# hpcaitech/Open-Sora

Hardware: NVIDIA H100
Metric: denoise-steps/sec STDiT3-XL/2 64x32x32 bf16 (higher is better)
Workload: dtype bf16

## Files before the change

### open-sora_b200/csrc/gemm_sm90.cu

```cuda
#include <stdlib.h>

#include <type_traits>

#include "common.cuh"
#include "tiles.cuh"
#include "wgmma.cuh"

namespace osb {

constexpr int kBlockM = 128;
constexpr int kBlockK = 64;
constexpr int kNumThreads = 384;
constexpr int kStageBudget = 200 * 1024;
constexpr int kSmemLimit = 227 * 1024;

enum { kPlain = 0, kConv = 1, kHeadTiles = 2, kLora = 3, kText = 4, kFp8 = 5, kFp8Blk = 6 };

struct Fp8BlockParams {
  int64_t a_ld, a_kstride;
  uint8_t* d8;
  float* d_scale;
  int64_t ldd8, ld_dscale;
};

// ... 23 lines not shown
  const float* sin;
};

struct ConvGeom {
  int32_t wt_log2, ht_log2;
  int32_t tiles_w, tiles_h, tiles_t, nb;
  int32_t w_out, h_out, t_out;
  int32_t sw, sh, st;
  int32_t kw_n, kh_n;
  int32_t cin_chunks;
};

__host__ __device__ constexpr bool staged_epilogue(int mode) { return mode == kPlain || mode == kConv || mode == kLora || mode == kFp8 || mode == kFp8Blk; }

template <int BLOCK_N, bool kStaged = false>
struct GemmCfg {
  static constexpr int A_BYTES = kBlockM * kBlockK * 2;
  static constexpr int B_BYTES = BLOCK_N * kBlockK * 2;
  static constexpr int STAGE_BYTES = A_BYTES + B_BYTES;
  static constexpr int EPI_BYTES = kStaged ? kBlockM * BLOCK_N * 2 : 0;
  static constexpr int RING_BUDGET = kStaged ? kSmemLimit - 1024 - 256 - EPI_BYTES : kStageBudget;
  static constexpr int STAGES_RAW = RING_BUDGET / STAGE_BYTES;
  static constexpr int STAGES = STAGES_RAW > 6 ? 6 : STAGES_RAW;
  static constexpr int NUM_BARS = 2 * STAGES + (kStaged ? 1 : 0);
  static constexpr int SMEM_BYTES = STAGES * STAGE_BYTES + EPI_BYTES + 1024 + 8 * NUM_BARS;
  static_assert(STAGES >= 2, "pipeline needs at least two stages");
  static_assert(SMEM_BYTES <= kSmemLimit, "shared memory");
  static_assert(B_BYTES % 1024 == 0, "W tile must keep 1024-byte swizzle-atom alignment");
  static_assert(BLOCK_N % 16 == 0 && BLOCK_N <= 256, "wgmma N");
  static_assert(!kStaged || BLOCK_N % 64 == 0, "the staged epilogue moves 64-column boxes");
};

template <int BLOCK_N, int kMode>
__global__ void __launch_bounds__(kNumThreads, 1)
gemm_bf16_kernel(const __grid_constant__ CUtensorMap tmap_a, const __grid_constant__ CUtensorMap tmap_w,
                 const GemmEpilogueParams p, const ConvGeom cg, const HeadTileParams ht,
                 const __grid_constant__ CUtensorMap tmap_u, const __grid_constant__ CUtensorMap tmap_lb,
                 const int32_t lora_k_blocks,
                 const float* a_scale, const float* w_scale,
                 const Fp8BlockParams fb,
                 const __grid_constant__ CUtensorMap tmap_r,
                 const __grid_constant__ CUtensorMap tmap_d) {
  constexpr bool kStaged = staged_epilogue(kMode);
  using Cfg = GemmCfg<BLOCK_N, kStaged>;
  constexpr int kStages = Cfg::STAGES;
  constexpr int kBK = (kMode == kFp8 || kMode == kFp8Blk) ? 2 * kBlockK : kBlockK;
  constexpr uint32_t kEpiBoxBytes = kBlockM * 128;

  extern __shared__ uint8_t smem_raw[];
  const uint32_t smem_base = (smem_u32(smem_raw) + 1023u) & ~1023u;
  const uint32_t epi_base = smem_base + kStages * Cfg::STAGE_BYTES;
  const uint32_t bar_base = epi_base + Cfg::EPI_BYTES;
  auto full_bar = [&](int s) { return bar_base + 8u * s; };
  auto empty_bar = [&](int s) { return bar_base + 8u * (kStages + s); };
  const uint32_t res_bar = bar_base + 8u * (2 * kStages);
  auto smem_a = [&](int s) { return smem_base + s * Cfg::STAGE_BYTES; };
  auto smem_b = [&](int s) { return smem_base + s * Cfg::STAGE_BYTES + Cfg::A_BYTES; };

  const int wg = threadIdx.x >> 7;
  const int tid_wg = threadIdx.x & 127;
  const int64_t num_n_blocks = (p.N + BLOCK_N - 1) / BLOCK_N;
  const int64_t m_blk = blockIdx.x / num_n_blocks, n_blk = blockIdx.x % num_n_blocks;
  const int64_t num_k_blocks = (p.K + kBK - 1) / kBK;
  const int64_t total_k_blocks = kMode == kLora ? num_k_blocks + lora_k_blocks : num_k_blocks;
  int n_i = 0, t0 = 0, h0 = 0, w0 = 0;
  if constexpr (kMode == kConv) {
    const int tw = (int)(m_blk % cg.tiles_w);
    const int th = (int)((m_blk / cg.tiles_w) % cg.tiles_h);
    const int tt = (int)((m_blk / ((int64_t)cg.tiles_w * cg.tiles_h)) % cg.tiles_t);
    n_i = (int)(m_blk / ((int64_t)cg.tiles_w * cg.tiles_h * cg.tiles_t));
    w0 = tw << cg.wt_log2;
    h0 = th << cg.ht_log2;
    t0 = tt * (128 >> (cg.wt_log2 + cg.ht_log2));
  }

  if (threadIdx.x == 0) {
    tma_prefetch_desc(&tmap_a);
    tma_prefetch_desc(&tmap_w);
    if constexpr (kMode == kLora) {
      tma_prefetch_desc(&tmap_u);
      tma_prefetch_desc(&tmap_lb);
    }
    if constexpr (kStaged) {
      if (p.R != nullptr) tma_prefetch_desc(&tmap_r);
      tma_prefetch_desc(&tmap_d);
      mbar_init(res_bar, 1);
    }
    for (int s = 0; s < kStages; ++s) {
      mbar_init(full_bar(s), 1);
      mbar_init(empty_bar(s), 2);
    }
    fence_barrier_init();
  }
  __syncthreads();
  pdl_wait();

  if (wg == 0) {
    if (tid_wg == 0) {
      const int32_t a_row = (int32_t)(m_blk * kBlockM);
      const int32_t w_row = (int32_t)(n_blk * BLOCK_N);
      if constexpr (kStaged) {
        if (p.R != nullptr) {
          const int live = (int)min((int64_t)(BLOCK_N / 64), (p.N - w_row + 63) / 64);
          mbar_expect_tx(res_bar, (uint32_t)live * kEpiBoxBytes);
          for (int c = 0; c < live; ++c) {
            if constexpr (kMode == kConv)
              tma_load_5d(&tmap_r, res_bar, epi_base + c * kEpiBoxBytes, w_row + 64 * c, w0, h0, t0, n_i);
            else
              tma_load_2d(&tmap_r, res_bar, epi_base + c * kEpiBoxBytes, w_row + 64 * c, a_row);
          }
        }
      }
      int stage = 0;
      uint32_t phase = 0;
      for (int64_t kb = 0; kb < num_k_blocks; ++kb) {
        mbar_wait_notrace(empty_bar(stage), phase ^ 1);
        const int32_t k0 = (int32_t)(kb * kBK);
        mbar_expect_tx(full_bar(stage), Cfg::STAGE_BYTES);
        if constexpr (kMode == kConv) {
          const int tap = (int)(kb / cg.cin_chunks);
          const int32_t ac = (int32_t)(kb - (int64_t)tap * cg.cin_chunks) * kBlockK;
          const int32_t aw = w0 * cg.sw + tap % cg.kw_n;
          const int32_t ah = h0 * cg.sh + (tap / cg.kw_n) % cg.kh_n;
          const int32_t at = t0 * cg.st + tap / (cg.kw_n * cg.kh_n);
          tma_load_5d(&tmap_a, full_bar(stage), smem_a(stage), ac, aw, ah, at, n_i);
        } else {
          tma_load_2d(&tmap_a, full_bar(stage), smem_a(stage), k0, a_row);
        }
        tma_load_2d(&tmap_w, full_bar(stage), smem_b(stage), k0, w_row);
        if (++stage == kStages) { stage = 0; phase ^= 1; }
      }
      if constexpr (kMode == kLora) {
        for (int32_t lk = 0; lk < lora_k_blocks; ++lk) {
          mbar_wait_notrace(empty_bar(stage), phase ^ 1);
          mbar_expect_tx(full_bar(stage), Cfg::STAGE_BYTES);
          tma_load_2d(&tmap_u, full_bar(stage), smem_a(stage), lk * kBlockK, a_row);
          tma_load_2d(&tmap_lb, full_bar(stage), smem_b(stage), lk * kBlockK, w_row);
          if (++stage == kStages) { stage = 0; phase ^= 1; }
        }
      }
      pdl_launch_dependents();
    }
    return;
  }

  const int cw = wg - 1;
  float acc[BLOCK_N / 2];
#pragma unroll
  for (int i = 0; i < BLOCK_N / 2; ++i) acc[i] = 0.f;
  if constexpr (kMode == kFp8 || kMode == kFp8Blk) {
    float part[BLOCK_N / 2];
#pragma unroll
    for (int i = 0; i < BLOCK_N / 2; ++i) part[i] = 0.f;
    const float* sa_row0 = a_scale;
    const float* sa_row1 = a_scale;
    if constexpr (kMode == kFp8Blk) {
      const int64_t r0 = m_blk * kBlockM + cw * 64 + (tid_wg >> 5) * 16 + ((tid_wg & 31) >> 2);
      sa_row0 = a_scale + min(r0, p.M - 1) * fb.a_ld;
      sa_row1 = a_scale + min(r0 + 8, p.M - 1) * fb.a_ld;
    }
    int stage = 0;
    uint32_t phase = 0;
    for (int64_t kb = 0; kb < total_k_blocks; ++kb) {
      float s0 = 1.f, s1 = 1.f;
      if constexpr (kMode == kFp8Blk) {
        s0 = __ldg(sa_row0 + kb * fb.a_kstride);
        s1 = __ldg(sa_row1 + kb * fb.a_kstride);
      }
      mbar_wait_notrace(full_bar(stage), phase);
      const uint64_t da = make_sw128_kmajor_desc(smem_a(stage) + (uint32_t)(cw * 64 * 128));
      const uint64_t db = make_sw128_kmajor_desc(smem_b(stage));
      wgmma_fence_regs(part);
      wgmma_fence();
#pragma unroll
      for (int k = 0; k < 4; ++k)
        WgmmaFp8<BLOCK_N>::mma(part, da + (uint64_t)(2 * k), db + (uint64_t)(2 * k), k > 0 ? 1u : 0u);
      wgmma_commit();
      wgmma_wait<0>();
      wgmma_fence_regs(part);
      if (tid_wg == 0) mbar_arrive(empty_bar(stage));
      if constexpr (kMode == kFp8Blk) {
#pragma unroll
        for (int j = 0; j < BLOCK_N / 8; ++j) {
          acc[4 * j] = fmaf(part[4 * j], s0, acc[4 * j]);
          acc[4 * j + 1] = fmaf(part[4 * j + 1], s0, acc[4 * j + 1]);
          acc[4 * j + 2] = fmaf(part[4 * j + 2], s1, acc[4 * j + 2]);
          acc[4 * j + 3] = fmaf(part[4 * j + 3], s1, acc[4 * j + 3]);
        }
      } else {
#pragma unroll
        for (int i = 0; i < BLOCK_N / 2; ++i) acc[i] += part[i];
      }
      if (++stage == kStages) { stage = 0; phase ^= 1; }
    }
  } else {
    int stage = 0, prev = 0;
    uint32_t phase = 0;
    for (int64_t kb = 0; kb < total_k_blocks; ++kb) {
      mbar_wait_notrace(full_bar(stage), phase);
      const uint64_t da = make_sw128_kmajor_desc(smem_a(stage) + (uint32_t)(cw * 64 * 128));
      const uint64_t db = make_sw128_kmajor_desc(smem_b(stage));
      wgmma_fence_regs(acc);
      wgmma_fence();
#pragma unroll
      for (int k = 0; k < kBlockK / 16; ++k)
        Wgmma<BLOCK_N>::mma(acc, da + (uint64_t)(2 * k), db + (uint64_t)(2 * k), (kb > 0 || k > 0) ? 1u : 0u);
      wgmma_commit();
      wgmma_wait<1>();
      wgmma_fence_regs(acc);
      if (kb > 0 && tid_wg == 0) mbar_arrive(empty_bar(prev));
      prev = stage;
      if (++stage == kStages) { stage = 0; phase ^= 1; }
    }
    wgmma_wait<0>();
    wgmma_fence_regs(acc);
  }

  const int warp_in = tid_wg >> 5, lane = tid_wg & 31;
  const int r_frag = cw * 64 + warp_in * 16 + (lane >> 2);
  const int c_frag = 2 * (lane & 3);

  if constexpr (kMode == kLora) {
    if (w_scale != nullptr) {
#pragma unroll
      for (int j = 0; j < BLOCK_N / 8; ++j) {
        const int64_t n = min(n_blk * BLOCK_N + 8 * j + c_frag, p.N - 2);
        const float2 cs = __ldg(reinterpret_cast<const float2*>(w_scale + n));
        acc[4 * j] *= cs.x;
        acc[4 * j + 1] *= cs.y;
        acc[4 * j + 2] *= cs.x;
        acc[4 * j + 3] *= cs.y;
      }
    }
  }

  if constexpr (kMode == kFp8Blk && BLOCK_N == 128) {
    if (p.epilogue == OSB_EPI_BIAS_GELU_TANH_FP8) {
      const int64_t n0 = n_blk * BLOCK_N + c_frag;
#pragma unroll
      for (int h = 0; h < 2; ++h) {
        const int64_t row = m_blk * kBlockM + r_frag + 8 * h;
        float amax = 0.f;
#pragma unroll
        for (int j = 0; j < BLOCK_N / 8; ++j) {
          const int64_t n = n0 + 8 * j;
          const float2 sw = __ldg(reinterpret_cast<const float2*>(w_scale + n));
          float v0 = acc[4 * j + 2 * h] * sw.x, v1 = acc[4 * j + 2 * h + 1] * sw.y;
          if (p.bias) {
            const float2 b = unpack_bf16x2(__ldg(reinterpret_cast<const uint32_t*>(p.bias + n)));
            v0 += b.x;
            v1 += b.y;
          }
          v0 = gelu_tanh(v0);
          v1 = gelu_tanh(v1);
          acc[4 * j + 2 * h] = v0;
          acc[4 * j + 2 * h + 1] = v1;
          amax = fmaxf(amax, fmaxf(fabsf(v0), fabsf(v1)));
        }
        amax = fmaxf(amax, __shfl_xor_sync(0xffffffffu, amax, 1));
        amax = fmaxf(amax, __shfl_xor_sync(0xffffffffu, amax, 2));
        const float s = amax > 0.f ? amax / 448.0f : 1.0f;
        if (row < p.M) {
          uint8_t* drow = fb.d8 + row * fb.ldd8;
#pragma unroll
          for (int j = 0; j < BLOCK_N / 8; ++j)
            *reinterpret_cast<uint16_t*>(drow + n0 + 8 * j) =
                (uint16_t)e4m3x2(acc[4 * j + 2 * h] / s, acc[4 * j + 2 * h + 1] / s);
          if (c_frag == 0) fb.d_scale[row * fb.ld_dscale + n_blk] = s;
        }
      }
      return;
    }
  }

  if constexpr (kMode == kHeadTiles) {
    constexpr int D = BLOCK_N / 2;
    using HT = HeadTileCfg<D>;
    constexpr int JH = D / 8;
    const int C = ht.heads * D;
    const uint32_t chunk_bytes = (uint32_t)ht.map.TR * 128u;
#pragma unroll
    for (int h = 0; h < 2; ++h) {
      const int64_t row = m_blk * kBlockM + r_frag + 8 * h;
      const bool row_ok = row < p.M;
      uint32_t pos = 0, tile_i = 0;
      int r = 0;
      if (row_ok) tile_of_row(ht.map, (uint32_t)row, tile_i, pos, r);
#pragma unroll
      for (int hh = 0; hh < 2; ++hh) {
        const int64_t col0 = n_blk * BLOCK_N + hh * D;
        if (col0 >= p.N) continue;
        const int kidx = (int)((uint32_t)col0 / (uint32_t)C);
        const int head = (int)((uint32_t)col0 - (uint32_t)kidx * (uint32_t)C) / D;
        const int kind = kidx % ht.nkinds;
        float x[JH][2];
#pragma unroll
        for (int j = 0; j < JH; ++j) {
          x[j][0] = acc[4 * (hh * JH + j) + 2 * h];
          x[j][1] = acc[4 * (hh * JH + j) + 2 * h + 1];
          if (p.bias) {
            const float2 b = unpack_bf16x2(__ldg(reinterpret_cast<const uint32_t*>(p.bias + col0 + 8 * j + c_frag)));
            x[j][0] += b.x;
            x[j][1] += b.y;
          }
        }
        if ((ht.norm_mask >> kind) & 1u) {
          float ss = 0.f;
#pragma unroll
          for (int j = 0; j < JH; ++j) ss += x[j][0] * x[j][0] + x[j][1] * x[j][1];
          ss += __shfl_xor_sync(0xffffffffu, ss, 1);
          ss += __shfl_xor_sync(0xffffffffu, ss, 2);
          const float rs = rsqrtf(ss * (1.0f / D) + ht.eps);
          const __nv_bfloat16* w = kind == 0 ? ht.norm_w[0] : (kind == 1 ? ht.norm_w[1] : (kind == 2 ? ht.norm_w[2] : ht.norm_w[3]));
#pragma unroll
          for (int j = 0; j < JH; ++j) {
            const float2 f = unpack_bf16x2(__ldg(reinterpret_cast<const uint32_t*>(w + 8 * j + c_frag)));
            x[j][0] *= rs * f.x;
            x[j][1] *= rs * f.y;
          }
        }
        if (!row_ok) continue;
        if ((ht.rope_mask >> kind) & 1u) {
#pragma unroll
          for (int j = 0; j < JH; ++j) {
            const int64_t i = (int64_t)pos * (D / 2) + (8 * j + c_frag) / 2;
            const float cc = __ldg(ht.cos + i), sn = __ldg(ht.sin + i);
            const float a = x[j][0], b = x[j][1];
            x[j][0] = a * cc - b * sn;
            x[j][1] = b * cc + a * sn;
          }
        }
        uint8_t* dst = ht.base + (int64_t)kidx * ht.kind_stride + (int64_t)head * ht.head_stride + (int64_t)tile_i * ht.tile_bytes;
#pragma unroll
        for (int j = 0; j < JH; ++j)
          *reinterpret_cast<uint32_t*>(dst + tile_unit_off<HT::MAIN>(r, j, chunk_bytes) + c_frag * 2) = pack_bf16x2(x[j][0], x[j][1]);
        if constexpr (HT::UP > HT::U)
          *reinterpret_cast<uint32_t*>(dst + tile_unit_off<HT::MAIN>(r, HT::U, chunk_bytes) + c_frag * 2) = 0u;
      }
    }
  } else if constexpr (kMode == kText) {
#pragma unroll
    for (int h = 0; h < 2; ++h) {
      const int64_t row = m_blk * kBlockM + r_frag + 8 * h;
      if (row >= p.M) continue;
      __nv_bfloat16* drow = p.D + row * p.ldd;
#pragma unroll
      for (int j = 0; j < BLOCK_N / 8; ++j) {
        const int64_t n = n_blk * BLOCK_N + 8 * j + c_frag;
        if (n >= p.N) continue;
        float v0 = acc[4 * j + 2 * h], v1 = acc[4 * j + 2 * h + 1];
        if (p.bias) {
          const float2 b = unpack_bf16x2(__ldg(reinterpret_cast<const uint32_t*>(p.bias + n)));
          v0 += b.x;
          v1 += b.y;
        }
        if (p.epilogue == OSB_EPI_GATED_GELU) {
          drow[n >> 1] = __float2bfloat16_rn(gelu_tanh(v0) * v1);
        } else {
          v0 = v0 / (1.0f + __expf(-1.702f * v0));
          v1 = v1 / (1.0f + __expf(-1.702f * v1));
          *reinterpret_cast<uint32_t*>(drow + n) = pack_bf16x2(v0, v1);
        }
      }
    }
  } else {
    static_assert(kStaged, "every other mode has its own epilogue");
    const float* gate_row[2] = {nullptr, nullptr};
    float sa[2] = {0.f, 0.f};
    if constexpr (kMode != kConv) {
      const uint32_t group_rows32 = (uint32_t)(p.group_rows > 0xffffffffll ? 0xffffffffu : p.group_rows);
#pragma unroll
      for (int h = 0; h < 2; ++h) {
        const int64_t row = min(m_blk * kBlockM + r_frag + 8 * h, p.M - 1);
        if (p.epilogue == OSB_EPI_BIAS_GATE_RES && p.gate != nullptr) {
          int64_t gi = (uint32_t)row / group_rows32;
          if (p.mod_index) gi = p.mod_index[gi];
          gate_row[h] = p.gate + gi * p.gate_stride;
        }
        if constexpr (kMode == kFp8) sa[h] = __ldg(a_scale + row);
      }
    }
    uint8_t* const epi = smem_raw + (epi_base - smem_u32(smem_raw));
    const bool gate_res = p.epilogue == OSB_EPI_BIAS_GATE_RES;
    if (!gate_res) gate_row[0] = gate_row[1] = nullptr;
    const bool has_res = gate_res && p.R != nullptr;
    if (p.R != nullptr) mbar_wait_notrace(res_bar, 0);
    auto body = [&](auto gelu) {
#pragma unroll
      for (int j = 0; j < BLOCK_N / 8; ++j) {
        const int64_t n = min(n_blk * BLOCK_N + 8 * j + c_frag, p.N - 2);
        float2 sw = make_float2(1.f, 1.f), b = make_float2(-0.f, -0.f);
        if constexpr (kMode == kFp8 || kMode == kFp8Blk) sw = __ldg(reinterpret_cast<const float2*>(w_scale + n));
        if (p.bias) b = unpack_bf16x2(__ldg(reinterpret_cast<const uint32_t*>(p.bias + n)));
#pragma unroll
        for (int h = 0; h < 2; ++h) {
          const int li = r_frag + 8 * h;
          uint32_t* const cell = reinterpret_cast<uint32_t*>(epi + (j >> 3) * kEpiBoxBytes + li * 128 +
                                                             (((j & 7) ^ (li & 7)) << 4) + c_frag * 2);
          float v0 = acc[4 * j + 2 * h], v1 = acc[4 * j + 2 * h + 1];
          if constexpr (kMode == kFp8) {
            v0 = __fmul_rn(v0, __fmul_rn(sa[h], sw.x));
            v1 = __fmul_rn(v1, __fmul_rn(sa[h], sw.y));
          } else if constexpr (kMode == kFp8Blk) {
            v0 = __fmul_rn(v0, sw.x);
            v1 = __fmul_rn(v1, sw.y);
          }
          v0 = __fadd_rn(v0, b.x);
          v1 = __fadd_rn(v1, b.y);
          if constexpr (decltype(gelu)::value) {
            v0 = gelu_tanh(v0);
            v1 = gelu_tanh(v1);
          } else {
            const float2 g = gate_row[h] ? __ldg(reinterpret_cast<const float2*>(gate_row[h] + n)) : make_float2(1.f, 1.f);
            const float2 rv = has_res ? unpack_bf16x2(*cell) : make_float2(-0.f, -0.f);
            v0 = __fadd_rn(__fmul_rn(v0, g.x), rv.x);
            v1 = __fadd_rn(__fmul_rn(v1, g.y), rv.y);
          }
          *cell = pack_bf16x2(v0, v1);
        }
      }
    };
    if (p.epilogue == OSB_EPI_BIAS_GELU_TANH)
      body(std::true_type{});
    else
      body(std::false_type{});
    fence_proxy_async_smem();
    named_barrier_sync(1, 256);
    if (threadIdx.x == 128) {
      const int32_t n0 = (int32_t)(n_blk * BLOCK_N);
      const int live = (int)min((int64_t)(BLOCK_N / 64), (p.N - n0 + 63) / 64);
      for (int c = 0; c < live; ++c) {
        if constexpr (kMode == kConv)
          tma_store_5d(&tmap_d, epi_base + c * kEpiBoxBytes, n0 + 64 * c, w0, h0, t0, n_i);
        else
          tma_store_2d(&tmap_d, epi_base + c * kEpiBoxBytes, n0 + 64 * c, (int32_t)(m_blk * kBlockM));
      }
      bulk_commit_group();
      bulk_wait_group_read_all();
    }
  }
}

template <int BLOCK_N, int kMode>
static int launch_kernel(const CUtensorMap& ta, const CUtensorMap& tw, const GemmEpilogueParams& p, const ConvGeom& cg,
                         const HeadTileParams& ht, int64_t tiles, cudaStream_t stream, const CUtensorMap* tu = nullptr,
                         const CUtensorMap* tlb = nullptr, int32_t lora_k_blocks = 0, const float* a_scale = nullptr,
                         const float* w_scale = nullptr, const Fp8BlockParams& fb = Fp8BlockParams{},
                         const CUtensorMap* tr = nullptr, const CUtensorMap* td = nullptr) {
  if (tiles >= (1ll << 31)) { set_error("osb gemm: too many output tiles (%lld)", (long long)tiles); return OSB_ERR_UNSUPPORTED; }
  cudaLaunchAttribute attr[2];
  cudaLaunchConfig_t cfg = launch_config(dim3((unsigned)tiles), dim3(kNumThreads),
                                         GemmCfg<BLOCK_N, staged_epilogue(kMode)>::SMEM_BYTES, stream, attr);
  OSB_CHECK_CUDA(cudaLaunchKernelEx(&cfg, gemm_bf16_kernel<BLOCK_N, kMode>, ta, tw, p, cg, ht, tu ? *tu : ta,
                                    tlb ? *tlb : tw, lora_k_blocks, a_scale, w_scale, fb, tr ? *tr : ta, td ? *td : ta));
  count_launch();
  return OSB_OK;
}

static int make_epilogue_maps(const GemmEpilogueParams& p, CUtensorMap* tr, CUtensorMap* td) {
  if (int rc = make_tmap_2d_bf16(td, p.D, p.M, p.N, p.ldd, kBlockM, 64)) return rc;
  if (p.R != nullptr) return make_tmap_2d_bf16(tr, p.R, p.M, p.N, p.ldr, kBlockM, 64);
  *tr = *td;
  return OSB_OK;
}

template <int D>
static int launch_gemm_ht(const osb_gemm_args& a, const HeadTileParams& ht, cudaStream_t stream) {
  constexpr int BLOCK_N = 2 * D;
  CUtensorMap ta, tw;
  int rc = make_tmap_2d_bf16(&ta, a.A, a.M, a.K, a.lda, kBlockM, kBlockK);
  if (rc) return rc;
  rc = make_tmap_2d_bf16(&tw, a.W, a.N, a.K, a.ldw, BLOCK_N, kBlockK);
  if (rc) return rc;
  GemmEpilogueParams p = {};
// ... 65 lines not shown
  if ((rc = init_one<128, kLora>())) return rc;
  if ((rc = init_one<192, kLora>())) return rc;
  if ((rc = init_one<256, kLora>())) return rc;
  if ((rc = init_one<64, kText>())) return rc;
  if ((rc = init_one<128, kText>())) return rc;
  if ((rc = init_one<192, kText>())) return rc;
  if ((rc = init_one<256, kText>())) return rc;
  if ((rc = init_one<64, kFp8>())) return rc;
  if ((rc = init_one<128, kFp8>())) return rc;
  if ((rc = init_one<64, kFp8Blk>())) return rc;
  if ((rc = init_one<128, kFp8Blk>())) return rc;
  return OSB_OK;
}

static int pick_block_n(int64_t M, int64_t N) {
  if (N <= 64) return 64;
  const int cands[3] = {256, 192, 128};
  int best = 256;
  int64_t best_cost = INT64_MAX;
  for (int i = 0; i < 3; ++i) {
    const int bn = cands[i];
    const int64_t tiles = ((M + kBlockM - 1) / kBlockM) * ((N + bn - 1) / bn);
    const int64_t waves = (tiles + sm_count() - 1) / sm_count();
    const int64_t cost = waves * bn;
    if (cost < best_cost) { best_cost = cost; best = bn; }
  }
  return best;
}

template <int BLOCK_N, int kMode = kFp8>
static int launch_gemm_fp8(const osb_gemm_fp8_args& a, cudaStream_t stream, const Fp8BlockParams& fb = Fp8BlockParams{}) {
  CUtensorMap ta, tw;
  int rc = make_tmap_2d_e4m3(&ta, a.A, a.M, a.K, a.lda, kBlockM, 2 * kBlockK);
  if (rc) return rc;
  rc = make_tmap_2d_e4m3(&tw, a.W, a.N, a.K, a.ldw, BLOCK_N, 2 * kBlockK);
  if (rc) return rc;
  GemmEpilogueParams p = {};
  p.bias = static_cast<const __nv_bfloat16*>(a.bias);
  p.D = static_cast<__nv_bfloat16*>(a.D);
  p.R = a.epilogue == OSB_EPI_BIAS_GATE_RES ? static_cast<const __nv_bfloat16*>(a.R) : nullptr;
  p.gate = a.gate;
  p.mod_index = a.mod_index;
  p.M = a.M; p.N = a.N; p.K = a.K;
  p.ldd = a.ldd;
  p.ldr = a.ldr;
  p.group_rows = a.group_rows > 0 ? a.group_rows : a.M;
  p.gate_stride = a.gate_stride;
// ... 302 lines not shown
```

Baseline: 11.20.

## Make SM90 GEMM persistent with overlapped epilogue and producer register rebalancing

Turns the one-tile-per-CTA GEMM into a persistent kernel: the grid is capped at the SM count and each CTA loops over tiles. The producer warp loads the next tile's K-blocks while the consumers run the previous epilogue, using a new epi_free barrier to guard the staged-epilogue buffer. The producer warpgroup gives up registers via setmaxnreg and the consumers take more. The head-tile epilogue now packs values with lane shuffles into 16-byte stores. The block-N cost model adds a per-tile overhead term. This hides launch and epilogue latency at the price of more synchronisation complexity and possible tile-scheduling imbalance.

Measured after the change: 11.94 (median of 6 runs). 6.6% higher.

```diff
diff --git a/open-sora_b200/csrc/gemm_sm90.cu b/open-sora_b200/csrc/gemm_sm90.cu
--- a/open-sora_b200/csrc/gemm_sm90.cu
+++ b/open-sora_b200/csrc/gemm_sm90.cu
@@ -69,7 +69,7 @@
   static constexpr int RING_BUDGET = kStaged ? kSmemLimit - 1024 - 256 - EPI_BYTES : kStageBudget;
   static constexpr int STAGES_RAW = RING_BUDGET / STAGE_BYTES;
   static constexpr int STAGES = STAGES_RAW > 6 ? 6 : STAGES_RAW;
-  static constexpr int NUM_BARS = 2 * STAGES + (kStaged ? 1 : 0);
+  static constexpr int NUM_BARS = 2 * STAGES + (kStaged ? 2 : 0);
   static constexpr int SMEM_BYTES = STAGES * STAGE_BYTES + EPI_BYTES + 1024 + 8 * NUM_BARS;
   static_assert(STAGES >= 2, "pipeline needs at least two stages");
   static_assert(SMEM_BYTES <= kSmemLimit, "shared memory");
@@ -101,25 +101,35 @@
   auto full_bar = [&](int s) { return bar_base + 8u * s; };
   auto empty_bar = [&](int s) { return bar_base + 8u * (kStages + s); };
   const uint32_t res_bar = bar_base + 8u * (2 * kStages);
+  const uint32_t epi_free = bar_base + 8u * (2 * kStages + 1);
   auto smem_a = [&](int s) { return smem_base + s * Cfg::STAGE_BYTES; };
   auto smem_b = [&](int s) { return smem_base + s * Cfg::STAGE_BYTES + Cfg::A_BYTES; };
 
   const int wg = threadIdx.x >> 7;
   const int tid_wg = threadIdx.x & 127;
   const int64_t num_n_blocks = (p.N + BLOCK_N - 1) / BLOCK_N;
-  const int64_t m_blk = blockIdx.x / num_n_blocks, n_blk = blockIdx.x % num_n_blocks;
+  const int64_t num_m_blocks =
+      kMode == kConv ? (int64_t)cg.nb * cg.tiles_t * cg.tiles_h * cg.tiles_w : (p.M + kBlockM - 1) / kBlockM;
+  const int64_t num_tiles = num_m_blocks * num_n_blocks;
   const int64_t num_k_blocks = (p.K + kBK - 1) / kBK;
   const int64_t total_k_blocks = kMode == kLora ? num_k_blocks + lora_k_blocks : num_k_blocks;
-  int n_i = 0, t0 = 0, h0 = 0, w0 = 0;
-  if constexpr (kMode == kConv) {
-    const int tw = (int)(m_blk % cg.tiles_w);
-    const int th = (int)((m_blk / cg.tiles_w) % cg.tiles_h);
-    const int tt = (int)((m_blk / ((int64_t)cg.tiles_w * cg.tiles_h)) % cg.tiles_t);
-    n_i = (int)(m_blk / ((int64_t)cg.tiles_w * cg.tiles_h * cg.tiles_t));
-    w0 = tw << cg.wt_log2;
-    h0 = th << cg.ht_log2;
-    t0 = tt * (128 >> (cg.wt_log2 + cg.ht_log2));
-  }
+  struct Tile {
+    int64_t m_blk, n_blk;
+    int n_i, t0, h0, w0;
+  };
+  auto tile_at = [&](int64_t t) {
+    Tile tl = {t / num_n_blocks, t % num_n_blocks, 0, 0, 0, 0};
+    if constexpr (kMode == kConv) {
+      const int tw = (int)(tl.m_blk % cg.tiles_w);
+      const int th = (int)((tl.m_blk / cg.tiles_w) % cg.tiles_h);
+      const int tt = (int)((tl.m_blk / ((int64_t)cg.tiles_w * cg.tiles_h)) % cg.tiles_t);
+      tl.n_i = (int)(tl.m_blk / ((int64_t)cg.tiles_w * cg.tiles_h * cg.tiles_t));
+      tl.w0 = tw << cg.wt_log2;
+      tl.h0 = th << cg.ht_log2;
+      tl.t0 = tt * (128 >> (cg.wt_log2 + cg.ht_log2));
+    }
+    return tl;
+  };
 
   if (threadIdx.x == 0) {
     tma_prefetch_desc(&tmap_a);
@@ -132,6 +142,7 @@
       if (p.R != nullptr) tma_prefetch_desc(&tmap_r);
       tma_prefetch_desc(&tmap_d);
       mbar_init(res_bar, 1);
+      mbar_init(epi_free, 1);
     }
     for (int s = 0; s < kStages; ++s) {
       mbar_init(full_bar(s), 1);
@@ -143,278 +154,82 @@
   pdl_wait();
 
   if (wg == 0) {
+    asm volatile("setmaxnreg.dec.sync.aligned.u32 40;\n" ::: "memory");
     if (tid_wg == 0) {
-      const int32_t a_row = (int32_t)(m_blk * kBlockM);
-      const int32_t w_row = (int32_t)(n_blk * BLOCK_N);
-      if constexpr (kStaged) {
-        if (p.R != nullptr) {
-          const int live = (int)min((int64_t)(BLOCK_N / 64), (p.N - w_row + 63) / 64);
-          mbar_expect_tx(res_bar, (uint32_t)live * kEpiBoxBytes);
-          for (int c = 0; c < live; ++c) {
-            if constexpr (kMode == kConv)
-              tma_load_5d(&tmap_r, res_bar, epi_base + c * kEpiBoxBytes, w_row + 64 * c, w0, h0, t0, n_i);
-            else
-              tma_load_2d(&tmap_r, res_bar, epi_base + c * kEpiBoxBytes, w_row + 64 * c, a_row);
-          }
-        }
-      }
       int stage = 0;
       uint32_t phase = 0;
-      for (int64_t kb = 0; kb < num_k_blocks; ++kb) {
-        mbar_wait_notrace(empty_bar(stage), phase ^ 1);
-        const int32_t k0 = (int32_t)(kb * kBK);
-        mbar_expect_tx(full_bar(stage), Cfg::STAGE_BYTES);
-        if constexpr (kMode == kConv) {
-          const int tap = (int)(kb / cg.cin_chunks);
-          const int32_t ac = (int32_t)(kb - (int64_t)tap * cg.cin_chunks) * kBlockK;
-          const int32_t aw = w0 * cg.sw + tap % cg.kw_n;
-          const int32_t ah = h0 * cg.sh + (tap / cg.kw_n) % cg.kh_n;
-          const int32_t at = t0 * cg.st + tap / (cg.kw_n * cg.kh_n);
-          tma_load_5d(&tmap_a, full_bar(stage), smem_a(stage), ac, aw, ah, at, n_i);
-        } else {
-          tma_load_2d(&tmap_a, full_bar(stage), smem_a(stage), k0, a_row);
-        }
-        tma_load_2d(&tmap_w, full_bar(stage), smem_b(stage), k0, w_row);
-        if (++stage == kStages) { stage = 0; phase ^= 1; }
-      }
-      if constexpr (kMode == kLora) {
-        for (int32_t lk = 0; lk < lora_k_blocks; ++lk) {
+      uint32_t it = 0;
+      for (int64_t t = blockIdx.x; t < num_tiles; t += gridDim.x, ++it) {
+        const Tile tl = tile_at(t);
+        const int32_t a_row = (int32_t)(tl.m_blk * kBlockM);
+        const int32_t w_row = (int32_t)(tl.n_blk * BLOCK_N);
+        auto load_k_block = [&](int64_t kb) {
           mbar_wait_notrace(empty_bar(stage), phase ^ 1);
           mbar_expect_tx(full_bar(stage), Cfg::STAGE_BYTES);
-          tma_load_2d(&tmap_u, full_bar(stage), smem_a(stage), lk * kBlockK, a_row);
-          tma_load_2d(&tmap_lb, full_bar(stage), smem_b(stage), lk * kBlockK, w_row);
+          if (kMode == kLora && kb >= num_k_blocks) {
+            const int32_t lk0 = (int32_t)(kb - num_k_blocks) * kBlockK;
+            tma_load_2d(&tmap_u, full_bar(stage), smem_a(stage), lk0, a_row);
+            tma_load_2d(&tmap_lb, full_bar(stage), smem_b(stage), lk0, w_row);
+          } else {
+            const int32_t k0 = (int32_t)(kb * kBK);
+            if constexpr (kMode == kConv) {
+              const int tap = (int)(kb / cg.cin_chunks);
+              const int32_t ac = (int32_t)(kb - (int64_t)tap * cg.cin_chunks) * kBlockK;
+              const int32_t aw = tl.w0 * cg.sw + tap % cg.kw_n;
+              const int32_t ah = tl.h0 * cg.sh + (tap / cg.kw_n) % cg.kh_n;
+              const int32_t at = tl.t0 * cg.st + tap / (cg.kw_n * cg.kh_n);
+              tma_load_5d(&tmap_a, full_bar(stage), smem_a(stage), ac, aw, ah, at, tl.n_i);
+            } else {
+              tma_load_2d(&tmap_a, full_bar(stage), smem_a(stage), k0, a_row);
+            }
+            tma_load_2d(&tmap_w, full_bar(stage), smem_b(stage), k0, w_row);
+          }
           if (++stage == kStages) { stage = 0; phase ^= 1; }
+        };
+        int64_t kb = 0;
+        if constexpr (kStaged) {
+          if (p.R != nullptr) {
+            for (; kb < min((int64_t)kStages, total_k_blocks); ++kb) load_k_block(kb);
+            if (it > 0) mbar_wait_notrace(epi_free, (it - 1) & 1u);
+            const int live = (int)min((int64_t)(BLOCK_N / 64), (p.N - w_row + 63) / 64);
+            mbar_expect_tx(res_bar, (uint32_t)live * kEpiBoxBytes);
+            for (int c = 0; c < live; ++c) {
+              if constexpr (kMode == kConv)
+                tma_load_5d(&tmap_r, res_bar, epi_base + c * kEpiBoxBytes, w_row + 64 * c, tl.w0, tl.h0, tl.t0, tl.n_i);
+              else
+                tma_load_2d(&tmap_r, res_bar, epi_base + c * kEpiBoxBytes, w_row + 64 * c, a_row);
+            }
+          }
         }
+        for (; kb < total_k_blocks; ++kb) load_k_block(kb);
       }
       pdl_launch_dependents();
     }
     return;
   }
 
+  asm volatile("setmaxnreg.inc.sync.aligned.u32 232;\n" ::: "memory");
   const int cw = wg - 1;
-  float acc[BLOCK_N / 2];
-#pragma unroll
-  for (int i = 0; i < BLOCK_N / 2; ++i) acc[i] = 0.f;
-  if constexpr (kMode == kFp8 || kMode == kFp8Blk) {
-    float part[BLOCK_N / 2];
-#pragma unroll
-    for (int i = 0; i < BLOCK_N / 2; ++i) part[i] = 0.f;
-    const float* sa_row0 = a_scale;
-    const float* sa_row1 = a_scale;
-    if constexpr (kMode == kFp8Blk) {
-      const int64_t r0 = m_blk * kBlockM + cw * 64 + (tid_wg >> 5) * 16 + ((tid_wg & 31) >> 2);
-      sa_row0 = a_scale + min(r0, p.M - 1) * fb.a_ld;
-      sa_row1 = a_scale + min(r0 + 8, p.M - 1) * fb.a_ld;
-    }
-    int stage = 0;
-    uint32_t phase = 0;
-    for (int64_t kb = 0; kb < total_k_blocks; ++kb) {
-      float s0 = 1.f, s1 = 1.f;
-      if constexpr (kMode == kFp8Blk) {
-        s0 = __ldg(sa_row0 + kb * fb.a_kstride);
-        s1 = __ldg(sa_row1 + kb * fb.a_kstride);
-      }
-      mbar_wait_notrace(full_bar(stage), phase);
-      const uint64_t da = make_sw128_kmajor_desc(smem_a(stage) + (uint32_t)(cw * 64 * 128));
-      const uint64_t db = make_sw128_kmajor_desc(smem_b(stage));
-      wgmma_fence_regs(part);
-      wgmma_fence();
-#pragma unroll
-      for (int k = 0; k < 4; ++k)
-        WgmmaFp8<BLOCK_N>::mma(part, da + (uint64_t)(2 * k), db + (uint64_t)(2 * k), k > 0 ? 1u : 0u);
-      wgmma_commit();
-      wgmma_wait<0>();
-      wgmma_fence_regs(part);
-      if (tid_wg == 0) mbar_arrive(empty_bar(stage));
-      if constexpr (kMode == kFp8Blk) {
-#pragma unroll
-        for (int j = 0; j < BLOCK_N / 8; ++j) {
-          acc[4 * j] = fmaf(part[4 * j], s0, acc[4 * j]);
-          acc[4 * j + 1] = fmaf(part[4 * j + 1], s0, acc[4 * j + 1]);
-          acc[4 * j + 2] = fmaf(part[4 * j + 2], s1, acc[4 * j + 2]);
-          acc[4 * j + 3] = fmaf(part[4 * j + 3], s1, acc[4 * j + 3]);
-        }
-      } else {
-#pragma unroll
-        for (int i = 0; i < BLOCK_N / 2; ++i) acc[i] += part[i];
-      }
-      if (++stage == kStages) { stage = 0; phase ^= 1; }
-    }
-  } else {
-    int stage = 0, prev = 0;
-    uint32_t phase = 0;
-    for (int64_t kb = 0; kb < total_k_blocks; ++kb) {
-      mbar_wait_notrace(full_bar(stage), phase);
-      const uint64_t da = make_sw128_kmajor_desc(smem_a(stage) + (uint32_t)(cw * 64 * 128));
-      const uint64_t db = make_sw128_kmajor_desc(smem_b(stage));
-      wgmma_fence_regs(acc);
-      wgmma_fence();
-#pragma unroll
-      for (int k = 0; k < kBlockK / 16; ++k)
-        Wgmma<BLOCK_N>::mma(acc, da + (uint64_t)(2 * k), db + (uint64_t)(2 * k), (kb > 0 || k > 0) ? 1u : 0u);
-      wgmma_commit();
-      wgmma_wait<1>();
-      wgmma_fence_regs(acc);
-      if (kb > 0 && tid_wg == 0) mbar_arrive(empty_bar(prev));
-      prev = stage;
-      if (++stage == kStages) { stage = 0; phase ^= 1; }
-    }
-    wgmma_wait<0>();
-    wgmma_fence_regs(acc);
-  }
-
-  const int warp_in = tid_wg >> 5, lane = tid_wg & 31;
-  const int r_frag = cw * 64 + warp_in * 16 + (lane >> 2);
-  const int c_frag = 2 * (lane & 3);
-
-  if constexpr (kMode == kLora) {
-    if (w_scale != nullptr) {
-#pragma unroll
-      for (int j = 0; j < BLOCK_N / 8; ++j) {
-        const int64_t n = min(n_blk * BLOCK_N + 8 * j + c_frag, p.N - 2);
-        const float2 cs = __ldg(reinterpret_cast<const float2*>(w_scale + n));
-        acc[4 * j] *= cs.x;
-        acc[4 * j + 1] *= cs.y;
-        acc[4 * j + 2] *= cs.x;
-        acc[4 * j + 3] *= cs.y;
-      }
-    }
-  }
-
-  if constexpr (kMode == kFp8Blk && BLOCK_N == 128) {
-    if (p.epilogue == OSB_EPI_BIAS_GELU_TANH_FP8) {
-      const int64_t n0 = n_blk * BLOCK_N + c_frag;
-#pragma unroll
-      for (int h = 0; h < 2; ++h) {
-        const int64_t row = m_blk * kBlockM + r_frag + 8 * h;
-        float amax = 0.f;
-#pragma unroll
-        for (int j = 0; j < BLOCK_N / 8; ++j) {
-          const int64_t n = n0 + 8 * j;
-          const float2 sw = __ldg(reinterpret_cast<const float2*>(w_scale + n));
-          float v0 = acc[4 * j + 2 * h] * sw.x, v1 = acc[4 * j + 2 * h + 1] * sw.y;
-          if (p.bias) {
-            const float2 b = unpack_bf16x2(__ldg(reinterpret_cast<const uint32_t*>(p.bias + n)));
-            v0 += b.x;
-            v1 += b.y;
-          }
-          v0 = gelu_tanh(v0);
-          v1 = gelu_tanh(v1);
-          acc[4 * j + 2 * h] = v0;
-          acc[4 * j + 2 * h + 1] = v1;
-          amax = fmaxf(amax, fmaxf(fabsf(v0), fabsf(v1)));
-        }
-        amax = fmaxf(amax, __shfl_xor_sync(0xffffffffu, amax, 1));
-        amax = fmaxf(amax, __shfl_xor_sync(0xffffffffu, amax, 2));
-        const float s = amax > 0.f ? amax / 448.0f : 1.0f;
-        if (row < p.M) {
-          uint8_t* drow = fb.d8 + row * fb.ldd8;
-#pragma unroll
-          for (int j = 0; j < BLOCK_N / 8; ++j)
-            *reinterpret_cast<uint16_t*>(drow + n0 + 8 * j) =
-                (uint16_t)e4m3x2(acc[4 * j + 2 * h] / s, acc[4 * j + 2 * h + 1] / s);
-          if (c_frag == 0) fb.d_scale[row * fb.ld_dscale + n_blk] = s;
-        }
-      }
-      return;
-    }
-  }
-
-  if constexpr (kMode == kHeadTiles) {
-    constexpr int D = BLOCK_N / 2;
-    using HT = HeadTileCfg<D>;
-    constexpr int JH = D / 8;
-    const int C = ht.heads * D;
-    const uint32_t chunk_bytes = (uint32_t)ht.map.TR * 128u;
-#pragma unroll
-    for (int h = 0; h < 2; ++h) {
-      const int64_t row = m_blk * kBlockM + r_frag + 8 * h;
-      const bool row_ok = row < p.M;
-      uint32_t pos = 0, tile_i = 0;
-      int r = 0;
-      if (row_ok) tile_of_row(ht.map, (uint32_t)row, tile_i, pos, r);
-#pragma unroll
-      for (int hh = 0; hh < 2; ++hh) {
-        const int64_t col0 = n_blk * BLOCK_N + hh * D;
-        if (col0 >= p.N) continue;
-        const int kidx = (int)((uint32_t)col0 / (uint32_t)C);
-        const int head = (int)((uint32_t)col0 - (uint32_t)kidx * (uint32_t)C) / D;
-        const int kind = kidx % ht.nkinds;
-        float x[JH][2];
-#pragma unroll
-        for (int j = 0; j < JH; ++j) {
-          x[j][0] = acc[4 * (hh * JH + j) + 2 * h];
-          x[j][1] = acc[4 * (hh * JH + j) + 2 * h + 1];
-          if (p.bias) {
-            const float2 b = unpack_bf16x2(__ldg(reinterpret_cast<const uint32_t*>(p.bias + col0 + 8 * j + c_frag)));
-            x[j][0] += b.x;
-            x[j][1] += b.y;
-          }
-        }
-        if ((ht.norm_mask >> kind) & 1u) {
-          float ss = 0.f;
-#pragma unroll
-          for (int j = 0; j < JH; ++j) ss += x[j][0] * x[j][0] + x[j][1] * x[j][1];
-          ss += __shfl_xor_sync(0xffffffffu, ss, 1);
-          ss += __shfl_xor_sync(0xffffffffu, ss, 2);
-          const float rs = rsqrtf(ss * (1.0f / D) + ht.eps);
-          const __nv_bfloat16* w = kind == 0 ? ht.norm_w[0] : (kind == 1 ? ht.norm_w[1] : (kind == 2 ? ht.norm_w[2] : ht.norm_w[3]));
-#pragma unroll
-          for (int j = 0; j < JH; ++j) {
-            const float2 f = unpack_bf16x2(__ldg(reinterpret_cast<const uint32_t*>(w + 8 * j + c_frag)));
-            x[j][0] *= rs * f.x;
-            x[j][1] *= rs * f.y;
-          }
-        }
-        if (!row_ok) continue;
-        if ((ht.rope_mask >> kind) & 1u) {
-#pragma unroll
-          for (int j = 0; j < JH; ++j) {
-            const int64_t i = (int64_t)pos * (D / 2) + (8 * j + c_frag) / 2;
-            const float cc = __ldg(ht.cos + i), sn = __ldg(ht.sin + i);
-            const float a = x[j][0], b = x[j][1];
-            x[j][0] = a * cc - b * sn;
-            x[j][1] = b * cc + a * sn;
-          }
-        }
-        uint8_t* dst = ht.base + (int64_t)kidx * ht.kind_stride + (int64_t)head * ht.head_stride + (int64_t)tile_i * ht.tile_bytes;
-#pragma unroll
-        for (int j = 0; j < JH; ++j)
-          *reinterpret_cast<uint32_t*>(dst + tile_unit_off<HT::MAIN>(r, j, chunk_bytes) + c_frag * 2) = pack_bf16x2(x[j][0], x[j][1]);
-        if constexpr (HT::UP > HT::U)
-          *reinterpret_cast<uint32_t*>(dst + tile_unit_off<HT::MAIN>(r, HT::U, chunk_bytes) + c_frag * 2) = 0u;
-      }
-    }
-  } else if constexpr (kMode == kText) {
-#pragma unroll
-    for (int h = 0; h < 2; ++h) {
-      const int64_t row = m_blk * kBlockM + r_frag + 8 * h;
-      if (row >= p.M) continue;
-      __nv_bfloat16* drow = p.D + row * p.ldd;
-#pragma unroll
-      for (int j = 0; j < BLOCK_N / 8; ++j) {
-        const int64_t n = n_blk * BLOCK_N + 8 * j + c_frag;
-        if (n >= p.N) continue;
-        float v0 = acc[4 * j + 2 * h], v1 = acc[4 * j + 2 * h + 1];
-        if (p.bias) {
-          const float2 b = unpack_bf16x2(__ldg(reinterpret_cast<const uint32_t*>(p.bias + n)));
-          v0 += b.x;
-          v1 += b.y;
-        }
-        if (p.epilogue == OSB_EPI_GATED_GELU) {
-          drow[n >> 1] = __float2bfloat16_rn(gelu_tanh(v0) * v1);
-        } else {
-          v0 = v0 / (1.0f + __expf(-1.702f * v0));
-          v1 = v1 / (1.0f + __expf(-1.702f * v1));
-          *reinterpret_cast<uint32_t*>(drow + n) = pack_bf16x2(v0, v1);
-        }
-      }
-    }
-  } else {
-    static_assert(kStaged, "every other mode has its own epilogue");
+  int stage = 0;
+  uint32_t phase = 0;
+  uint32_t it = 0;
+  auto release_epi_buffer = [&](int64_t kb) {
+    if constexpr (kStaged) {
+      if (kb == 0 && it > 0 && threadIdx.x == 128) {
+        bulk_wait_group_read_all();
+        mbar_arrive(epi_free);
+      }
+    }
+  };
+  for (int64_t t = blockIdx.x; t < num_tiles; t += gridDim.x, ++it) {
+    const Tile tl = tile_at(t);
+    const int64_t m_blk = tl.m_blk, n_blk = tl.n_blk;
+    const int warp_in = tid_wg >> 5, lane = tid_wg & 31;
+    const int r_frag = cw * 64 + warp_in * 16 + (lane >> 2);
+    const int c_frag = 2 * (lane & 3);
     const float* gate_row[2] = {nullptr, nullptr};
     float sa[2] = {0.f, 0.f};
-    if constexpr (kMode != kConv) {
+    if constexpr (kStaged && kMode != kConv) {
       const uint32_t group_rows32 = (uint32_t)(p.group_rows > 0xffffffffll ? 0xffffffffu : p.group_rows);
 #pragma unroll
       for (int h = 0; h < 2; ++h) {
@@ -427,64 +242,300 @@
         if constexpr (kMode == kFp8) sa[h] = __ldg(a_scale + row);
       }
     }
-    uint8_t* const epi = smem_raw + (epi_base - smem_u32(smem_raw));
-    const bool gate_res = p.epilogue == OSB_EPI_BIAS_GATE_RES;
-    if (!gate_res) gate_row[0] = gate_row[1] = nullptr;
-    const bool has_res = gate_res && p.R != nullptr;
-    if (p.R != nullptr) mbar_wait_notrace(res_bar, 0);
-    auto body = [&](auto gelu) {
-#pragma unroll
-      for (int j = 0; j < BLOCK_N / 8; ++j) {
-        const int64_t n = min(n_blk * BLOCK_N + 8 * j + c_frag, p.N - 2);
-        float2 sw = make_float2(1.f, 1.f), b = make_float2(-0.f, -0.f);
-        if constexpr (kMode == kFp8 || kMode == kFp8Blk) sw = __ldg(reinterpret_cast<const float2*>(w_scale + n));
-        if (p.bias) b = unpack_bf16x2(__ldg(reinterpret_cast<const uint32_t*>(p.bias + n)));
+    float acc[BLOCK_N / 2];
+#pragma unroll
+    for (int i = 0; i < BLOCK_N / 2; ++i) acc[i] = 0.f;
+    if constexpr (kMode == kFp8 || kMode == kFp8Blk) {
+      float part[BLOCK_N / 2];
+#pragma unroll
+      for (int i = 0; i < BLOCK_N / 2; ++i) part[i] = 0.f;
+      const float* sa_row0 = a_scale;
+      const float* sa_row1 = a_scale;
+      if constexpr (kMode == kFp8Blk) {
+        const int64_t r0 = m_blk * kBlockM + cw * 64 + (tid_wg >> 5) * 16 + ((tid_wg & 31) >> 2);
+        sa_row0 = a_scale + min(r0, p.M - 1) * fb.a_ld;
+        sa_row1 = a_scale + min(r0 + 8, p.M - 1) * fb.a_ld;
+      }
+      for (int64_t kb = 0; kb < total_k_blocks; ++kb) {
+        float s0 = 1.f, s1 = 1.f;
+        if constexpr (kMode == kFp8Blk) {
+          s0 = __ldg(sa_row0 + kb * fb.a_kstride);
+          s1 = __ldg(sa_row1 + kb * fb.a_kstride);
+        }
+        mbar_wait_notrace(full_bar(stage), phase);
+        const uint64_t da = make_sw128_kmajor_desc(smem_a(stage) + (uint32_t)(cw * 64 * 128));
+        const uint64_t db = make_sw128_kmajor_desc(smem_b(stage));
+        wgmma_fence_regs(part);
+        wgmma_fence();
+#pragma unroll
+        for (int k = 0; k < 4; ++k)
+          WgmmaFp8<BLOCK_N>::mma(part, da + (uint64_t)(2 * k), db + (uint64_t)(2 * k), k > 0 ? 1u : 0u);
+        wgmma_commit();
+        release_epi_buffer(kb);
+        wgmma_wait<0>();
+        wgmma_fence_regs(part);
+        if (tid_wg == 0) mbar_arrive(empty_bar(stage));
+        if constexpr (kMode == kFp8Blk) {
+#pragma unroll
+          for (int j = 0; j < BLOCK_N / 8; ++j) {
+            acc[4 * j] = fmaf(part[4 * j], s0, acc[4 * j]);
+            acc[4 * j + 1] = fmaf(part[4 * j + 1], s0, acc[4 * j + 1]);
+            acc[4 * j + 2] = fmaf(part[4 * j + 2], s1, acc[4 * j + 2]);
+            acc[4 * j + 3] = fmaf(part[4 * j + 3], s1, acc[4 * j + 3]);
+          }
+        } else {
+#pragma unroll
+          for (int i = 0; i < BLOCK_N / 2; ++i) acc[i] += part[i];
+        }
+        if (++stage == kStages) { stage = 0; phase ^= 1; }
+      }
+    } else {
+      int prev = 0;
+      for (int64_t kb = 0; kb < total_k_blocks; ++kb) {
+        mbar_wait_notrace(full_bar(stage), phase);
+        const uint64_t da = make_sw128_kmajor_desc(smem_a(stage) + (uint32_t)(cw * 64 * 128));
+        const uint64_t db = make_sw128_kmajor_desc(smem_b(stage));
+        wgmma_fence_regs(acc);
+        wgmma_fence();
+#pragma unroll
+        for (int k = 0; k < kBlockK / 16; ++k)
+          Wgmma<BLOCK_N>::mma(acc, da + (uint64_t)(2 * k), db + (uint64_t)(2 * k), (kb > 0 || k > 0) ? 1u : 0u);
+        wgmma_commit();
+        release_epi_buffer(kb);
+        wgmma_wait<1>();
+        wgmma_fence_regs(acc);
+        if (kb > 0 && tid_wg == 0) mbar_arrive(empty_bar(prev));
+        prev = stage;
+        if (++stage == kStages) { stage = 0; phase ^= 1; }
+      }
+      wgmma_wait<0>();
+      wgmma_fence_regs(acc);
+      if (tid_wg == 0) mbar_arrive(empty_bar(prev));
+    }
+
+    if constexpr (kMode == kLora) {
+      if (w_scale != nullptr) {
+#pragma unroll
+        for (int j = 0; j < BLOCK_N / 8; ++j) {
+          const int64_t n = min(n_blk * BLOCK_N + 8 * j + c_frag, p.N - 2);
+          const float2 cs = __ldg(reinterpret_cast<const float2*>(w_scale + n));
+          acc[4 * j] *= cs.x;
+          acc[4 * j + 1] *= cs.y;
+          acc[4 * j + 2] *= cs.x;
+          acc[4 * j + 3] *= cs.y;
+        }
+      }
+    }
+
+    if constexpr (kMode == kFp8Blk && BLOCK_N == 128) {
+      if (p.epilogue == OSB_EPI_BIAS_GELU_TANH_FP8) {
+        const int64_t n0 = n_blk * BLOCK_N + c_frag;
 #pragma unroll
         for (int h = 0; h < 2; ++h) {
-          const int li = r_frag + 8 * h;
-          uint32_t* const cell = reinterpret_cast<uint32_t*>(epi + (j >> 3) * kEpiBoxBytes + li * 128 +
-                                                             (((j & 7) ^ (li & 7)) << 4) + c_frag * 2);
-          float v0 = acc[4 * j + 2 * h], v1 = acc[4 * j + 2 * h + 1];
-          if constexpr (kMode == kFp8) {
-            v0 = __fmul_rn(v0, __fmul_rn(sa[h], sw.x));
-            v1 = __fmul_rn(v1, __fmul_rn(sa[h], sw.y));
-          } else if constexpr (kMode == kFp8Blk) {
-            v0 = __fmul_rn(v0, sw.x);
-            v1 = __fmul_rn(v1, sw.y);
-          }
-          v0 = __fadd_rn(v0, b.x);
-          v1 = __fadd_rn(v1, b.y);
-          if constexpr (decltype(gelu)::value) {
+          const int64_t row = m_blk * kBlockM + r_frag + 8 * h;
+          float amax = 0.f;
+#pragma unroll
+          for (int j = 0; j < BLOCK_N / 8; ++j) {
+            const int64_t n = n0 + 8 * j;
+            const float2 sw = __ldg(reinterpret_cast<const float2*>(w_scale + n));
+            float v0 = acc[4 * j + 2 * h] * sw.x, v1 = acc[4 * j + 2 * h + 1] * sw.y;
+            if (p.bias) {
+              const float2 b = unpack_bf16x2(__ldg(reinterpret_cast<const uint32_t*>(p.bias + n)));
+              v0 += b.x;
+              v1 += b.y;
+            }
             v0 = gelu_tanh(v0);
             v1 = gelu_tanh(v1);
+            acc[4 * j + 2 * h] = v0;
+            acc[4 * j + 2 * h + 1] = v1;
+            amax = fmaxf(amax, fmaxf(fabsf(v0), fabsf(v1)));
+          }
+          amax = fmaxf(amax, __shfl_xor_sync(0xffffffffu, amax, 1));
+          amax = fmaxf(amax, __shfl_xor_sync(0xffffffffu, amax, 2));
+          const float s = amax > 0.f ? amax / 448.0f : 1.0f;
+          if (row < p.M) {
+            uint8_t* drow = fb.d8 + row * fb.ldd8;
+#pragma unroll
+            for (int j = 0; j < BLOCK_N / 8; ++j)
+              *reinterpret_cast<uint16_t*>(drow + n0 + 8 * j) =
+                  (uint16_t)e4m3x2(acc[4 * j + 2 * h] / s, acc[4 * j + 2 * h + 1] / s);
+            if (c_frag == 0) fb.d_scale[row * fb.ld_dscale + n_blk] = s;
+          }
+        }
+        continue;
+      }
+    }
+
+    if constexpr (kMode == kHeadTiles) {
+      constexpr int D = BLOCK_N / 2;
+      using HT = HeadTileCfg<D>;
+      constexpr int JH = D / 8;
+      const int C = ht.heads * D;
+      const uint32_t chunk_bytes = (uint32_t)ht.map.TR * 128u;
+#pragma unroll
+      for (int h = 0; h < 2; ++h) {
+        const int64_t row = m_blk * kBlockM + r_frag + 8 * h;
+        const bool row_ok = row < p.M;
+        uint32_t pos = 0, tile_i = 0;
+        int r = 0;
+        if (row_ok) tile_of_row(ht.map, (uint32_t)row, tile_i, pos, r);
+#pragma unroll
+        for (int hh = 0; hh < 2; ++hh) {
+          const int64_t col0 = n_blk * BLOCK_N + hh * D;
+          if (col0 >= p.N) continue;
+          const int kidx = (int)((uint32_t)col0 / (uint32_t)C);
+          const int head = (int)((uint32_t)col0 - (uint32_t)kidx * (uint32_t)C) / D;
+          const int kind = kidx % ht.nkinds;
+          float x[JH][2];
+#pragma unroll
+          for (int j = 0; j < JH; ++j) {
+            x[j][0] = acc[4 * (hh * JH + j) + 2 * h];
+            x[j][1] = acc[4 * (hh * JH + j) + 2 * h + 1];
+            if (p.bias) {
+              const float2 b = unpack_bf16x2(__ldg(reinterpret_cast<const uint32_t*>(p.bias + col0 + 8 * j + c_frag)));
+              x[j][0] += b.x;
+              x[j][1] += b.y;
+            }
+          }
+          if ((ht.norm_mask >> kind) & 1u) {
+            float ss = 0.f;
+#pragma unroll
+            for (int j = 0; j < JH; ++j) ss += x[j][0] * x[j][0] + x[j][1] * x[j][1];
+            ss += __shfl_xor_sync(0xffffffffu, ss, 1);
+            ss += __shfl_xor_sync(0xffffffffu, ss, 2);
+            const float rs = rsqrtf(ss * (1.0f / D) + ht.eps);
+            const __nv_bfloat16* w = kind == 0 ? ht.norm_w[0] : (kind == 1 ? ht.norm_w[1] : (kind == 2 ? ht.norm_w[2] : ht.norm_w[3]));
+#pragma unroll
+            for (int j = 0; j < JH; ++j) {
+              const float2 f = unpack_bf16x2(__ldg(reinterpret_cast<const uint32_t*>(w + 8 * j + c_frag)));
+              x[j][0] *= rs * f.x;
+              x[j][1] *= rs * f.y;
+            }
+          }
+          if ((ht.rope_mask >> kind) & 1u) {
+#pragma unroll
+            for (int j = 0; j < JH; ++j) {
+              const int64_t i = (int64_t)pos * (D / 2) + (8 * j + c_frag) / 2;
+              const float cc = __ldg(ht.cos + i), sn = __ldg(ht.sin + i);
+              const float a = x[j][0], b = x[j][1];
+              x[j][0] = a * cc - b * sn;
+              x[j][1] = b * cc + a * sn;
+            }
+          }
+          uint8_t* dst = ht.base + (int64_t)kidx * ht.kind_stride + (int64_t)head * ht.head_stride + (int64_t)tile_i * ht.tile_bytes;
+          const bool odd = (lane & 1) != 0, high = (lane & 2) != 0;
+#pragma unroll
+          for (int j0 = 0; j0 < HT::MAIN * 8; j0 += 4) {
+            uint32_t u0 = pack_bf16x2(x[j0][0], x[j0][1]), u1 = pack_bf16x2(x[j0 + 1][0], x[j0 + 1][1]);
+            uint32_t u2 = pack_bf16x2(x[j0 + 2][0], x[j0 + 2][1]), u3 = pack_bf16x2(x[j0 + 3][0], x[j0 + 3][1]);
+            uint32_t s0 = __shfl_xor_sync(0xffffffffu, odd ? u0 : u1, 1);
+            uint32_t s1 = __shfl_xor_sync(0xffffffffu, odd ? u2 : u3, 1);
+            if (odd) { u0 = s0; u2 = s1; } else { u1 = s0; u3 = s1; }
+            s0 = __shfl_xor_sync(0xffffffffu, high ? u0 : u2, 2);
+            s1 = __shfl_xor_sync(0xffffffffu, high ? u1 : u3, 2);
+            if (high) { u0 = s0; u1 = s1; } else { u2 = s0; u3 = s1; }
+            if (row_ok)
+              *reinterpret_cast<uint4*>(dst + tile_unit_off<HT::MAIN>(r, j0 + (lane & 3), chunk_bytes)) = make_uint4(u0, u1, u2, u3);
+          }
+          if (!row_ok) continue;
+#pragma unroll
+          for (int j = HT::MAIN * 8; j < JH; ++j)
+            *reinterpret_cast<uint32_t*>(dst + tile_unit_off<HT::MAIN>(r, j, chunk_bytes) + c_frag * 2) = pack_bf16x2(x[j][0], x[j][1]);
+          if constexpr (HT::UP > HT::U)
+            *reinterpret_cast<uint32_t*>(dst + tile_unit_off<HT::MAIN>(r, HT::U, chunk_bytes) + c_frag * 2) = 0u;
+        }
+      }
+    } else if constexpr (kMode == kText) {
+#pragma unroll
+      for (int h = 0; h < 2; ++h) {
+        const int64_t row = m_blk * kBlockM + r_frag + 8 * h;
+        if (row >= p.M) continue;
+        __nv_bfloat16* drow = p.D + row * p.ldd;
+#pragma unroll
+        for (int j = 0; j < BLOCK_N / 8; ++j) {
+          const int64_t n = n_blk * BLOCK_N + 8 * j + c_frag;
+          if (n >= p.N) continue;
+          float v0 = acc[4 * j + 2 * h], v1 = acc[4 * j + 2 * h + 1];
+          if (p.bias) {
+            const float2 b = unpack_bf16x2(__ldg(reinterpret_cast<const uint32_t*>(p.bias + n)));
+            v0 += b.x;
+            v1 += b.y;
+          }
+          if (p.epilogue == OSB_EPI_GATED_GELU) {
+            drow[n >> 1] = __float2bfloat16_rn(gelu_tanh(v0) * v1);
           } else {
-            const float2 g = gate_row[h] ? __ldg(reinterpret_cast<const float2*>(gate_row[h] + n)) : make_float2(1.f, 1.f);
-            const float2 rv = has_res ? unpack_bf16x2(*cell) : make_float2(-0.f, -0.f);
-            v0 = __fadd_rn(__fmul_rn(v0, g.x), rv.x);
-            v1 = __fadd_rn(__fmul_rn(v1, g.y), rv.y);
-          }
-          *cell = pack_bf16x2(v0, v1);
+            v0 = v0 / (1.0f + __expf(-1.702f * v0));
+            v1 = v1 / (1.0f + __expf(-1.702f * v1));
+            *reinterpret_cast<uint32_t*>(drow + n) = pack_bf16x2(v0, v1);
+          }
         }
       }
-    };
-    if (p.epilogue == OSB_EPI_BIAS_GELU_TANH)
-      body(std::true_type{});
-    else
-      body(std::false_type{});
-    fence_proxy_async_smem();
-    named_barrier_sync(1, 256);
-    if (threadIdx.x == 128) {
-      const int32_t n0 = (int32_t)(n_blk * BLOCK_N);
-      const int live = (int)min((int64_t)(BLOCK_N / 64), (p.N - n0 + 63) / 64);
-      for (int c = 0; c < live; ++c) {
-        if constexpr (kMode == kConv)
-          tma_store_5d(&tmap_d, epi_base + c * kEpiBoxBytes, n0 + 64 * c, w0, h0, t0, n_i);
-        else
-          tma_store_2d(&tmap_d, epi_base + c * kEpiBoxBytes, n0 + 64 * c, (int32_t)(m_blk * kBlockM));
-      }
-      bulk_commit_group();
-      bulk_wait_group_read_all();
-    }
+    } else {
+      static_assert(kStaged, "every other mode has its own epilogue");
+      uint8_t* const epi = smem_raw + (epi_base - smem_u32(smem_raw));
+      const bool gate_res = p.epilogue == OSB_EPI_BIAS_GATE_RES;
+      if (!gate_res) gate_row[0] = gate_row[1] = nullptr;
+      const bool has_res = gate_res && p.R != nullptr;
+      if (p.R != nullptr)
+        mbar_wait_notrace(res_bar, it & 1u);
+      else if (it > 0)
+        mbar_wait_notrace(epi_free, (it - 1) & 1u);
+      auto body = [&](auto gelu) {
+#pragma unroll
+        for (int j = 0; j < BLOCK_N / 8; ++j) {
+          const int64_t n = min(n_blk * BLOCK_N + 8 * j + c_frag, p.N - 2);
+          float2 sw = make_float2(1.f, 1.f), b = make_float2(-0.f, -0.f);
+          if constexpr (kMode == kFp8 || kMode == kFp8Blk) sw = __ldg(reinterpret_cast<const float2*>(w_scale + n));
+          if (p.bias) b = unpack_bf16x2(__ldg(reinterpret_cast<const uint32_t*>(p.bias + n)));
+#pragma unroll
+          for (int h = 0; h < 2; ++h) {
+            const int li = r_frag + 8 * h;
+            uint32_t* const cell = reinterpret_cast<uint32_t*>(epi + (j >> 3) * kEpiBoxBytes + li * 128 +
+                                                               (((j & 7) ^ (li & 7)) << 4) + c_frag * 2);
+            float v0 = acc[4 * j + 2 * h], v1 = acc[4 * j + 2 * h + 1];
+            if constexpr (kMode == kFp8) {
+              v0 = __fmul_rn(v0, __fmul_rn(sa[h], sw.x));
+              v1 = __fmul_rn(v1, __fmul_rn(sa[h], sw.y));
+            } else if constexpr (kMode == kFp8Blk) {
+              v0 = __fmul_rn(v0, sw.x);
+              v1 = __fmul_rn(v1, sw.y);
+            }
+            v0 = __fadd_rn(v0, b.x);
+            v1 = __fadd_rn(v1, b.y);
+            if constexpr (decltype(gelu)::value) {
+              v0 = gelu_tanh(v0);
+              v1 = gelu_tanh(v1);
+            } else {
+              const float2 g = gate_row[h] ? __ldg(reinterpret_cast<const float2*>(gate_row[h] + n)) : make_float2(1.f, 1.f);
+              const float2 rv = has_res ? unpack_bf16x2(*cell) : make_float2(-0.f, -0.f);
+              v0 = __fadd_rn(__fmul_rn(v0, g.x), rv.x);
+              v1 = __fadd_rn(__fmul_rn(v1, g.y), rv.y);
+            }
+            *cell = pack_bf16x2(v0, v1);
+          }
+        }
+      };
+      if (p.epilogue == OSB_EPI_BIAS_GELU_TANH)
+        body(std::true_type{});
+      else
+        body(std::false_type{});
+      fence_proxy_async_smem();
+      named_barrier_sync(1, 256);
+      if (threadIdx.x == 128) {
+        const int32_t n0 = (int32_t)(n_blk * BLOCK_N);
+        const int live = (int)min((int64_t)(BLOCK_N / 64), (p.N - n0 + 63) / 64);
+        for (int c = 0; c < live; ++c) {
+          if constexpr (kMode == kConv)
+            tma_store_5d(&tmap_d, epi_base + c * kEpiBoxBytes, n0 + 64 * c, tl.w0, tl.h0, tl.t0, tl.n_i);
+          else
+            tma_store_2d(&tmap_d, epi_base + c * kEpiBoxBytes, n0 + 64 * c, (int32_t)(m_blk * kBlockM));
+        }
+        bulk_commit_group();
+      }
+    }
+  }
+  if constexpr (kStaged) {
+    if (threadIdx.x == 128) bulk_wait_group_read_all();
   }
 }
 
@@ -495,8 +546,9 @@
                          const float* w_scale = nullptr, const Fp8BlockParams& fb = Fp8BlockParams{},
                          const CUtensorMap* tr = nullptr, const CUtensorMap* td = nullptr) {
   if (tiles >= (1ll << 31)) { set_error("osb gemm: too many output tiles (%lld)", (long long)tiles); return OSB_ERR_UNSUPPORTED; }
+  const int64_t grid = tiles < sm_count() ? tiles : sm_count();
   cudaLaunchAttribute attr[2];
-  cudaLaunchConfig_t cfg = launch_config(dim3((unsigned)tiles), dim3(kNumThreads),
+  cudaLaunchConfig_t cfg = launch_config(dim3((unsigned)grid), dim3(kNumThreads),
                                          GemmCfg<BLOCK_N, staged_epilogue(kMode)>::SMEM_BYTES, stream, attr);
   OSB_CHECK_CUDA(cudaLaunchKernelEx(&cfg, gemm_bf16_kernel<BLOCK_N, kMode>, ta, tw, p, cg, ht, tu ? *tu : ta,
                                     tlb ? *tlb : tw, lora_k_blocks, a_scale, w_scale, fb, tr ? *tr : ta, td ? *td : ta));
@@ -608,7 +660,7 @@
     const int bn = cands[i];
     const int64_t tiles = ((M + kBlockM - 1) / kBlockM) * ((N + bn - 1) / bn);
     const int64_t waves = (tiles + sm_count() - 1) / sm_count();
-    const int64_t cost = waves * bn;
+    const int64_t cost = waves * (bn + 16);
     if (cost < best_cost) { best_cost = cost; best = bn; }
   }
   return best;
```
